# cryscan/bevy-hikari

Hardware: NVIDIA H100
Metric: Mrays/s (higher is better)
Workload: dtype f32

## Files before the change

bevy_hikari_b200/csrc/hk_device.cuh:

```cuda
#pragma once
#include <cuda_runtime.h>
#include <stdint.h>

#include "hikari_b200.h"
#include "hk_math.h"

#ifndef HK_INL_PACK
#define HK_INL_PACK __forceinline__
#endif
#ifndef HK_INL_TRAVERSE
#define HK_INL_TRAVERSE __forceinline__
#endif
#ifndef HK_INL_HITINFO
#define HK_INL_HITINFO __forceinline__
#endif
#ifndef HK_INL_TEXTURE
#define HK_INL_TEXTURE __forceinline__
#endif
#ifndef HK_SURFACE_LOOP
#define HK_SURFACE_LOOP 0
#endif
#ifndef HK_INL_SURFACE
#define HK_INL_SURFACE __forceinline__
#endif
// ... 516 lines not shown
        const uint32_t id0 = __float_as_uint(t0.x), id1 = __float_as_uint(t1.x), id2 = __float_as_uint(t1.w), id3 = __float_as_uint(t2.z);
#pragma unroll 1
        for (int k = 0; k < 4; ++k) {
            const uint32_t id = k == 0 ? id0 : (k == 1 ? id1 : (k == 2 ? id2 : id3));
            if (id == U32_MAX) continue;
            const vec4 t = sample_texture(sc, id, uv);
            if (k == 0) s.base_color = s.base_color * t;
            else if (k == 1) s.emissive = s.emissive * t;
            else if (k == 2) s.metallic *= t.x;
            else s.occlusion = t.x;
        }
#else
        uint32_t id = __float_as_uint(t0.x);
        if (id != U32_MAX) s.base_color = s.base_color * sample_texture(sc, id, uv);
        id = __float_as_uint(t1.x);
        if (id != U32_MAX) s.emissive = s.emissive * sample_texture(sc, id, uv);
        id = __float_as_uint(t1.w);
        if (id != U32_MAX) s.metallic *= sample_texture(sc, id, uv).x;
        id = __float_as_uint(t2.z);
        if (id != U32_MAX) s.occlusion = sample_texture(sc, id, uv).x;
#endif
    }
    s.roughness = perceptualRoughnessToRoughness(t1.y);
    s.reflectance = t2.x;
    return s;
}
static __device__ HK_INL_SURFACE vec4 retreive_emissive(const DeviceScene& sc, uint32_t material_index, vec2 uv) {
    const float4* m = reinterpret_cast<const float4*>(sc.materials + material_index);
    vec4 emissive = f4v(ldg4(m + 2));
    if (sc.texture_count != 0u) {
        uint32_t id = __float_as_uint(ldg4(m + 3).x);
        if (id != U32_MAX) emissive = emissive * sample_texture(sc, id, uv);
    }
    return emissive;
}

struct ShadeEnv {
    vec3 sun_dir; float cos_solar; vec3 sun_color; vec3 ambient; vec3 eye; bool ortho; vec3 ortho_dir;
};
__device__ __forceinline__ ShadeEnv make_env(const KParams& P) {
    ShadeEnv e;
    e.sun_dir = v3(P.in.lights.direction_to_light[0], P.in.lights.direction_to_light[1], P.in.lights.direction_to_light[2]);
    e.cos_solar = P.cos_solar_angle;
    e.sun_color = v3(P.in.lights.directional_color[0], P.in.lights.directional_color[1], P.in.lights.directional_color[2]);
    e.ambient = v3(P.in.lights.ambient_color[0], P.in.lights.ambient_color[1], P.in.lights.ambient_color[2]);
    e.eye = v3(P.in.view.world_position[0], P.in.view.world_position[1], P.in.view.world_position[2]);
    e.ortho = P.in.view.projection[15] == 1.0f;
    e.ortho_dir = v3(P.in.view.view_proj[2], P.in.view.view_proj[6], P.in.view.view_proj[10]);
    return e;
}
__device__ __forceinline__ vec3 calculate_view(const ShadeEnv& e, vec3 world_position) {
    return e.ortho ? normalize(e.ortho_dir) : normalize(e.eye - world_position);
}
__device__ __forceinline__ vec3 env_terms(vec3 diffuse_color, vec3 F0, float roughness, float NdotV) {
    return EnvBRDFApprox(diffuse_color, 1.0f, NdotV) + EnvBRDFApprox(F0, roughness, NdotV);
}
static __device__ HK_INL_SHADE vec3 env_brdf(vec3 V, vec3 N, const Surface& s) {
    vec3 base_color = xyz(s.base_color);
    float NdotV = fmax_(dot(N, V), 0.0001f);
    vec3 F0 = v3(0.16f * s.reflectance * s.reflectance * (1.0f - s.metallic)) + base_color * s.metallic;
    vec3 diffuse_color = base_color * (1.0f - s.metallic);
    return s.occlusion * env_terms(diffuse_color, F0, s.roughness, NdotV);
}
struct ShadeCtx {
    vec3 V, N, F0, diffuse_color, ambient_radiance;
    float roughness, NdotV, f90;
};
__device__ __forceinline__ ShadeCtx make_shade_ctx(const ShadeEnv& e, vec3 V, vec3 N, const Surface& s) {
    ShadeCtx c;
    vec3 base_color = xyz(s.base_color);
    c.V = V; c.N = N;
    c.F0 = v3(0.16f * s.reflectance * s.reflectance * (1.0f - s.metallic)) + base_color * s.metallic;
    c.diffuse_color = base_color * (1.0f - s.metallic);
    c.roughness = s.roughness;
    c.NdotV = fmax_(dot(N, V), 0.0001f);
    c.f90 = saturate(dot(c.F0, v3(50.0f * 0.33f)));
    c.ambient_radiance = s.occlusion * env_terms(c.diffuse_color, c.F0, s.roughness, c.NdotV) * e.ambient;
    return c;
}
__device__ __forceinline__ vec3 shade(const ShadeCtx& c, vec3 Lv, vec4 in_radiance) {
    vec3 Hv = normalize(Lv + c.V);
    float NoL = saturate(dot(c.N, Lv));
    float NoH = saturate(dot(c.N, Hv));
    float LoH = saturate(dot(Lv, Hv));
    vec3 diffuse = c.diffuse_color * Fd_Burley(c.roughness, c.NdotV, NoL, LoH);
    float D = D_GGX(c.roughness, NoH);
    float Vis = V_SmithGGXCorrelated(c.roughness, c.NdotV, NoL);
    vec3 F = F_Schlick_vec(c.F0, c.f90, LoH);
    vec3 specular_light = (1.0f * D * Vis) * F;
    vec3 lit_radiance = (specular_light + diffuse) * xyz(in_radiance) * NoL;
    return mix(lit_radiance, c.ambient_radiance, 1.0f - in_radiance.w);
}
static __device__ HK_INL_SHADE vec3 shading(const ShadeEnv& e, vec3 V, vec3 N, vec3 Lv, const Surface& s, vec4 in_radiance) {
    return shade(make_shade_ctx(e, V, N, s), Lv, in_radiance);
}
static __device__ HK_INL_RADIANCE vec4 input_radiance(const DeviceScene& sc, const ShadeEnv& e, vec3 ray_direction, const HitInfo& info,
                                               bool sample_directional, uint32_t sample_emissive, bool sample_ambient) {
    vec3 radiance = v3(0.0f);
    float amb = 0.0f;
    if (info.instance_index == U32_MAX) {
        bool hit_directional = dot(ray_direction, e.sun_dir) >= e.cos_solar;
        if (sample_directional && hit_directional) {
            radiance = e.sun_color;
        } else {
            radiance = sample_ambient ? e.ambient : v3(0.0f);
            amb = 1.0f;
        }
    } else if (sample_emissive == info.instance_index) {
        radiance = compute_emissive_radiance(retreive_emissive(sc, info.material_index, info.uv));
    }
    return v4(radiance, 1.0f - amb);
}

#ifndef HK_INL_WIDE
#define HK_INL_WIDE __forceinline__
#endif
template <bool BOTTOM>
static __device__ HK_INL_WIDE Hit wide_walk(const DeviceScene& sc, const Ray& ray, float max_distance, float early_distance,
                                            uint32_t exclude_instance, uint32_t instance);

template <bool COUNT_RAYS, bool WIDE = false>
static __device__ HK_INL_SELECT LightCandidate select_light_candidate(const DeviceScene& sc, const ShadeEnv& e, vec4 rnd, vec3 position,
                                                                 vec3 normal, uint32_t instance, HitInfo& info, uint32_t& blas_rays) {
    LightCandidate cand;
    cand.max_distance = F32_MAX;
    cand.min_distance = DISTANCE_MAX;
    cand.emissive_instance = DONT_SAMPLE_EMISSIVE;
    vec3 rand_direction = mul(normal_basis(e.sun_dir), sample_uniform_cone_dir(rnd.z, rnd.w, e.cos_solar));
    cand.direction = rand_direction;
    cand.p = 1.0f;
    info = empty_hit_info(position, rand_direction);
    if (instance == DONT_SAMPLE_EMISSIVE) return cand;

    uint32_t picked = U32_MAX;
    float count = 0.0f;
    float rand_1d = rnd.x;
    uint32_t index = 0;
    while (index < sc.emissive_node_count) {
        float4 n0 = ldg4(&sc.emissive_nodes[index]);
        uint32_t entry = __float_as_uint(n0.w);
        if (entry >= BVH_LEAF_FLAG) {
            uint32_t emissive_index = entry - BVH_LEAF_FLAG;
            float4 pr = ldg4(sc.emissives[emissive_index].position);
            uint32_t em_instance = __ldg(&sc.emissives[emissive_index].instance);
            vec3 c = f4xyz(pr);
            vec3 bmin = c - pr.w, bmax = c + pr.w;
            bool inside = position.x > bmin.x && position.y > bmin.y && position.z > bmin.z &&
                          position.x < bmax.x && position.y < bmax.y && position.z < bmax.z;
            if (instance != em_instance && inside) {
                rand_1d = fract(rand_1d + GOLDEN_RATIO);
                count += 1.0f;
                if (rand_1d < 1.0f / count) { cand.emissive_instance = em_instance; picked = emissive_index; }
            }
            index = __ldg(&sc.emissive_nodes[index].exit_index);
        } else {
            float4 n1 = ldg4(reinterpret_cast<const float4*>(&sc.emissive_nodes[index]) + 1);
            bool inside = position.x > n0.x && position.y > n0.y && position.z > n0.z &&
                          position.x < n1.x && position.y < n1.y && position.z < n1.z;
            index = inside ? entry : __float_as_uint(n1.w);
        }
    }

    if (cand.emissive_instance != DONT_SAMPLE_EMISSIVE) {
        const hk_emissive* em = sc.emissives + picked;
        uint4 e2 = ldg4u(&em->instance);
        float surface_area = __ldg(&em->surface_area);
        uint32_t alias_index = min(f32_to_u32(rnd.x * (float)e2.w), e2.w - 1u);
        uint2 ae = __ldg(reinterpret_cast<const uint2*>(sc.alias_table + e2.z + alias_index));
        uint32_t primitive_index = (rnd.y < __uint_as_float(ae.x)) ? ae.y : alias_index;

        const hk_instance* einst = sc.instances + cand.emissive_instance;
        uint4 mesh = ldg4u(&einst->mesh);
        const hk_primitive* prim = sc.primitives + mesh.y + primitive_index;
        vec3 p0 = f4xyz(ldg4(&prim->vertices[0])), p1 = f4xyz(ldg4(&prim->vertices[1])), p2 = f4xyz(ldg4(&prim->vertices[2]));
        float srx = sqrtf(rnd.z);
        float bx = 1.0f - srx, by = rnd.w * srx;
        vec3 lp = bx * p0 + by * p1 + (1.0f - bx - by) * p2;
        const float4* mm = reinterpret_cast<const float4*>(einst->model);
        mat4 model;
        model.c[0] = f4v(ldg4(mm)); model.c[1] = f4v(ldg4(mm + 1)); model.c[2] = f4v(ldg4(mm + 2)); model.c[3] = f4v(ldg4(mm + 3));
        vec4 wp = mul(model, v4(lp, 1.0f));
        vec3 p = xyz(wp) / wp.w;

        Hit hit;
        hit.u = 0.0f; hit.v = 0.0f; hit.distance = F32_MAX; hit.instance_index = U32_MAX; hit.primitive_index = U32_MAX;
        Ray ray;
        ray.origin = position + normal * RAY_BIAS;
        ray.direction = normalize(p - position);
        ray.inv_direction = v3(0.0f);
        cand.direction = ray.direction;
        bool found = false;
        if (dot(cand.direction, normal) > 0.0f) {
            if (COUNT_RAYS) blas_rays += 1u;
            Ray r;
            instance_ray(einst, ray, r);
            if constexpr (WIDE) {
                hit = wide_walk<true>(sc, r, F32_MAX, 0.0f, DONT_EXCLUDE, cand.emissive_instance);
                found = hit.primitive_index != U32_MAX;
            } else {
                found = traverse_bottom(sc, hit, r, mesh.y, mesh.z, mesh.w, 0.0f);
            }
        }
        if (found) {
            hit.instance_index = e2.x;
            info = hit_info(sc, ray, hit);
            cand.max_distance = hit.distance;
            cand.min_distance = hit.distance - 0.1f;
            vec3 delta = xyz(info.position) - position;
            cand.p = dot(delta, delta) / fabsf(dot(ray.direction, info.normal) * surface_area);
            cand.p = cand.p / count;
        } else {
            info = empty_hit_info(ray.origin, ray.direction);
            cand.emissive_instance = DONT_SAMPLE_EMISSIVE;
            cand.direction = rand_direction;
            cand.p = 1.0f;
        }
    }
    return cand;
}

__device__ __forceinline__ size_t band_index(const Band& b, int x, int y) { return (size_t)(y - b.a0) * (size_t)b.AW + (size_t)(x - b.ax0); }
__device__ __forceinline__ bool band_allocated(const Band& b, int x, int y) { return x >= b.ax0 && x < b.ax1 && y >= b.a0 && y < b.a1; }
__device__ __forceinline__ bool band_owned(const Band& b, int x, int y) { return x >= b.cx0 && x < b.cx1 && y >= b.r0 && y < b.r1; }
__device__ __forceinline__ size_t render_index(const Band& b, int x, int y) { return (size_t)(y - b.a0) * (size_t)b.RS + (size_t)(x - b.ax0); }
__device__ __forceinline__ size_t owned_index(const Band& b, int x, int y) { return (size_t)(y - b.r0) * (size_t)(b.cx1 - b.cx0) + (size_t)(x - b.cx0); }

__device__ __forceinline__ vec4 noise_random(const KParams& P, int x, int y) {
    uint32_t number = P.in.frame.number;
    uint32_t noise_id = number % NOISE_TEXTURE_COUNT;
    uint32_t tx = ((uint32_t)x + number) & 63u, ty = ((uint32_t)y + number) & 63u;
    uchar4 t = __ldg(reinterpret_cast<const uchar4*>(P.noise) + ((noise_id * 64u + ty) * 64u + tx));
    vec4 rnd = v4(unorm8(t.x), unorm8(t.y), unorm8(t.z), unorm8(t.w));
    return fract(rnd + (float)number * GOLDEN_RATIO);
}

__device__ __forceinline__ vec2 render_uv(const KParams& P, int x, int y) {
    return (v2((float)x, (float)y) + 0.5f) / v2((float)P.band.RW, (float)P.band.RH);
}
__device__ __forceinline__ vec2 jittered_deferred_uv(const KParams& P, vec2 uv, float amount) {
    if (P.ratio1) return uv;
    vec2 texel_size = v2(1.0f, 1.0f) / v2((float)P.band.W, (float)P.band.H);
    return uv + (P.jitter_sign * amount) * texel_size * P.ratio_m1;
}
__device__ __forceinline__ void light_deferred_coords(const KParams& P, vec2 uv, int x, int y, int& dx, int& dy) {
    if (P.ratio1) { dx = x; dy = y; return; }
    vec2 d = jittered_deferred_uv(P, uv, 0.25f);
    dx = f32_to_i32(d.x * (float)P.band.W); dy = f32_to_i32(d.y * (float)P.band.H);
}
__device__ __forceinline__ void denoise_deferred_coords(const KParams& P, vec2 uv, int x, int y, int& dx, int& dy) {
    if (P.ratio1) { dx = x; dy = y; return; }
    vec2 d = jittered_deferred_uv(P, uv, 0.5f);
    dx = min(max((int)floorf(d.x * (float)P.band.W), 0), P.band.W - 1);
    dy = min(max((int)floorf(d.y * (float)P.band.H), 0), P.band.H - 1);
}
__device__ __forceinline__ bool render_allocated(const KParams& P, int x, int y) {
    return P.ratio1 ? band_allocated(P.band, x, y) : (x >= 0 && x < P.band.RW && y >= 0 && y < P.band.RH);
}

struct PassBuffers {
    ReservoirPlanes previous_reservoir, reservoir, previous_spatial_reservoir, spatial_reservoir;
};
__device__ __forceinline__ PassBuffers bind(const KParams& P, int signal) {
    const int temporal = (signal == 0) ? 0 : (signal == 1 ? 2 : 6);
    const int spatial = (signal == 2) ? 8 : 4;
    const int current = (int)(P.in.frame.number & 1u), previous = 1 - current;
    PassBuffers b;
    b.previous_reservoir = P.planes.reservoir[current + temporal];
    b.reservoir = P.planes.reservoir[previous + temporal];
    b.previous_spatial_reservoir = P.planes.reservoir[current + spatial];
    b.spatial_reservoir = P.planes.reservoir[previous + spatial];
    return b;
}
__device__ __forceinline__ bool previous_pixel(const KParams& P, vec2 previous_uv, bool inclusive, size_t& pidx) {
    float ax = fabsf(previous_uv.x - 0.5f), ay = fabsf(previous_uv.y - 0.5f);
    bool inside = inclusive ? (ax <= 0.5f && ay <= 0.5f) : (ax < 0.5f && ay < 0.5f);
    if (!inside) return false;
    int px = f32_to_i32(previous_uv.x * (float)P.band.RW), py = f32_to_i32(previous_uv.y * (float)P.band.RH);
    if (!render_allocated(P, px, py)) return false;
    pidx = render_index(P.band, px, py);
    return true;
}
__device__ __forceinline__ vec2 pixel_uv(const KParams& P, int x, int y) { return render_uv(P, x, y); }
__device__ __forceinline__ size_t light_gbuffer_index(const KParams& P, int x, int y, size_t render_idx) {
    if (P.ratio1) return render_idx;
    int dx, dy;
    light_deferred_coords(P, render_uv(P, x, y), x, y, dx, dy);
    return band_index(P.band, dx, dy);
}

constexpr uint32_t SCATTER_BACKGROUND = 0u, SCATTER_MISS = 1u, SCATTER_VALIDATION = 2u;
__device__ __forceinline__ void scatter_claim(const KParams& P, size_t target, int x, int y, uint32_t kind) {
    uint32_t writer = (uint32_t)y * (uint32_t)P.band.RW + (uint32_t)x;
    atomicMax(&P.planes.scatter_key[target], ((writer + 1u) << 2) | kind);
}

#ifndef HK_CTA_WARPS
#define HK_CTA_WARPS 4
#endif
static_assert(HK_CTA_WARPS == 2 || HK_CTA_WARPS == 4 || HK_CTA_WARPS == 8, "tile_pixel places warps in pairs");
constexpr int TILE_W = 16, TILE_H = 2 * HK_CTA_WARPS, CTA_THREADS = 32 * HK_CTA_WARPS;
#ifndef HK_MINB_INDIRECT
#define HK_MINB_INDIRECT 8
#endif
#ifndef HK_MINB_DIRECT
#define HK_MINB_DIRECT 8
#endif
#ifndef HK_MINB_GBUFFER
#define HK_MINB_GBUFFER 8
#endif
#ifndef HK_MINB_INDIRECT_WIDE
#define HK_MINB_INDIRECT_WIDE 6
#endif
#ifndef HK_MINB_DIRECT_WIDE
#define HK_MINB_DIRECT_WIDE 6
#endif
#ifndef HK_MINB_DENOISE
#define HK_MINB_DENOISE 8
#endif
#ifndef HK_MINB_SPATIAL
#define HK_MINB_SPATIAL 8
#endif
__device__ __forceinline__ void tile_pixel(int& x, int& y, const KParams& P) {
    int lane = threadIdx.x & 31, warp = threadIdx.x >> 5;
    x = P.col_lo + blockIdx.x * TILE_W + (warp & 1) * 8 + (lane & 7);
    y = P.row_lo + blockIdx.y * TILE_H + (warp >> 1) * 4 + (lane >> 3);
}
__device__ __forceinline__ bool tile_active(const KParams& P, int x, int y) { return x < P.col_hi && y < P.row_hi; }

}
```

bevy_hikari_b200/csrc/kernels_light.cu:

```cuda
#include "hk_device.cuh"
#include "hk_wide.cuh"
#include "hk_kernels.h"

#ifndef HK_NO_TEXTURE_VARIANT
#define HK_NO_TEXTURE_VARIANT 1
#endif
#ifndef HK_NOVAL_VARIANT
#define HK_NOVAL_VARIANT 1
#endif

namespace hkd {

template <bool COUNT>
__device__ __forceinline__ void flush_counters(const KParams& P, uint32_t primary, uint32_t tlas, uint32_t blas) {
    if (!COUNT || P.counters == nullptr) return;
    for (int o = 16; o > 0; o >>= 1) {
        primary += __shfl_xor_sync(0xffffffffu, primary, o);
        tlas += __shfl_xor_sync(0xffffffffu, tlas, o);
        blas += __shfl_xor_sync(0xffffffffu, blas, o);
    }
    if ((threadIdx.x & 31) == 0) {
        if (primary) atomicAdd(&P.counters->primary, (unsigned long long)primary);
        if (tlas) atomicAdd(&P.counters->tlas, (unsigned long long)tlas);
        if (blas) atomicAdd(&P.counters->blas, (unsigned long long)blas);
    }
}

template <bool WIDE>
__device__ __forceinline__ Hit trace_top(const DeviceScene& sc, const Ray& ray, float max_distance, float early_distance, uint32_t exclude_instance) {
    if constexpr (WIDE) return wide_walk<false>(sc, ray, max_distance, early_distance, exclude_instance, 0u);
    else return traverse_top(sc, ray, max_distance, early_distance, exclude_instance);
}

__device__ __forceinline__ mat4 load_mat4(const float* m) {
    mat4 r;
    for (int c = 0; c < 4; ++c) r.c[c] = v4(m[4 * c], m[4 * c + 1], m[4 * c + 2], m[4 * c + 3]);
    return r;
}

__device__ __forceinline__ Ray primary_ray(const KParams& P, const mat4& inv_view_proj, float px, float py, vec2 jitter_ndc) {
    vec2 uv = v2(px + 0.5f, py + 0.5f) / v2((float)P.band.W, (float)P.band.H);
    vec2 ndc = v2(uv.x * 2.0f - 1.0f, (1.0f - uv.y) * 2.0f - 1.0f) - jitter_ndc;
    vec4 p = mul(inv_view_proj, v4(ndc.x, ndc.y, 1.0f, 1.0f));
    vec3 near_point = xyz(p) / p.w;
    Ray ray;
    if (P.in.view.projection[15] == 1.0f) {
        vec4 q = mul(inv_view_proj, v4(ndc.x, ndc.y, 0.0f, 1.0f));
        ray.origin = near_point;
        ray.direction = normalize(xyz(q) / q.w - near_point);
    } else {
        ray.origin = v3(P.in.view.world_position[0], P.in.view.world_position[1], P.in.view.world_position[2]);
        ray.direction = normalize(near_point - ray.origin);
    }
    ray.inv_direction = 1.0f / ray.direction;
    return ray;
}

template <bool TEX>
__device__ __forceinline__ DeviceScene scene_variant(const DeviceScene& scene) {
    DeviceScene sc = scene;
    if (!TEX) sc.texture_count = 0u;
    return sc;
}

template <bool COUNT, bool TEX = true, bool WIDE = false>
__global__ void __launch_bounds__(CTA_THREADS, HK_MINB_GBUFFER) k_gbuffer(const __grid_constant__ KParams P) {
    int x, y;
    tile_pixel(x, y, P);
    const bool active = tile_active(P, x, y);
    uint32_t n_primary = 0;
    if (active) {
        const size_t idx = band_index(P.band, x, y);
        const mat4 view_proj = load_mat4(P.in.view.view_proj);
        const mat4 inv_view_proj = load_mat4(P.in.view.inverse_view_proj);
        vec2 jitter_ndc = v2(0.0f, 0.0f);
        if (P.in.taa_jitter) {
            uint32_t index = P.in.smaa_tu4x ? ((P.in.frame.number >> 1u) & 15u) : (P.in.frame.number & 15u);
            const float* h = P.in.frame.halton[index >> 1u];
            vec2 hj = ((index & 1u) == 0u) ? v2(h[0], h[1]) : v2(h[2], h[3]);
            vec2 j = 2.0f * hj * (v2(1.0f, 1.0f) / v2(P.in.view.viewport[2], P.in.view.viewport[3]));
            jitter_ndc = v2(j.x, -j.y);
        }
        Ray ray = primary_ray(P, inv_view_proj, (float)x, (float)y, jitter_ndc);
        n_primary = 1;
        Hit hit = trace_top<WIDE>(P.scene, ray, F32_MAX, 0.0f, DONT_EXCLUDE);
        if (hit.instance_index == U32_MAX) {
            P.planes.pos_depth[idx] = make_float4(0.0f, 0.0f, 0.0f, 0.0f);
            P.planes.depth[idx] = 0.0f;
            P.planes.normal[idx] = 0u;
            P.planes.depth_gradient[idx] = make_float2(0.0f, 0.0f);
            P.planes.instance_material[idx] = make_float2(0.0f, 0.0f);
            P.planes.velocity_uv[idx] = make_float4(0.0f, 0.0f, 0.0f, 0.0f);
            P.planes.albedo[idx] = make_uint2(0u, 0u);
        } else {
            const DeviceScene sc = scene_variant<TEX>(P.scene);
            const hk_instance* inst = sc.instances + hit.instance_index;
            const hk_primitive* prim = sc.primitives + hit.primitive_index;
            uint32_t vbase = __ldg(&inst->mesh.vertex);
            uint32_t material = __ldg(&inst->material);
            float4 pa = ldg4(&prim->vertices[0]), pb = ldg4(&prim->vertices[1]), pc = ldg4(&prim->vertices[2]);
            const hk_vertex* va = sc.vertices + vbase + __float_as_uint(pa.w);
            const hk_vertex* vb = sc.vertices + vbase + __float_as_uint(pb.w);
            const hk_vertex* vc = sc.vertices + vbase + __float_as_uint(pc.w);
            float4 a0 = ldg4(va), a1 = ldg4(reinterpret_cast<const float4*>(va) + 1);
            float4 b0 = ldg4(vb), b1 = ldg4(reinterpret_cast<const float4*>(vb) + 1);
            float4 c0 = ldg4(vc), c1 = ldg4(reinterpret_cast<const float4*>(vc) + 1);
            vec3 world_position = ray.origin + ray.direction * hit.distance;
            vec4 clip = mul(view_proj, v4(world_position, 1.0f));
            float depth = clip.z / clip.w;
            vec3 n0 = instance_normal_local_to_world(inst, f4xyz(a1));
            vec3 n1 = instance_normal_local_to_world(inst, f4xyz(b1));
            vec3 n2 = instance_normal_local_to_world(inst, f4xyz(c1));
            vec3 world_normal = n0 + hit.u * (n1 - n0) + hit.v * (n2 - n0);
            vec2 uv0 = v2(a0.w, a1.w), uv1 = v2(b0.w, b1.w), uv2 = v2(c0.w, c1.w);
            vec2 tex_uv = uv0 + hit.u * (uv1 - uv0) + hit.v * (uv2 - uv0);
            const mat4 model = load_mat4(inst->model);
            vec3 P0 = xyz(mul(model, v4(f4xyz(pa), 1.0f)));
            vec3 P1 = xyz(mul(model, v4(f4xyz(pb), 1.0f)));
            vec3 P2 = xyz(mul(model, v4(f4xyz(pc), 1.0f)));
            vec3 Ng = cross(P1 - P0, P2 - P0);
            Ray rx = primary_ray(P, inv_view_proj, (float)x + 1.0f, (float)y, jitter_ndc);
            float tx = dot(P0 - rx.origin, Ng) / dot(rx.direction, Ng);
            vec4 cx = mul(view_proj, v4(rx.origin + rx.direction * tx, 1.0f));
            Ray ry = primary_ray(P, inv_view_proj, (float)x, (float)y + 1.0f, jitter_ndc);
            float ty = dot(P0 - ry.origin, Ng) / dot(ry.direction, Ng);
            vec4 cy = mul(view_proj, v4(ry.origin + ry.direction * ty, 1.0f));
            vec2 grad = v2(cx.z / cx.w - depth, cy.z / cy.w - depth);
            vec3 previous_world_position = world_position;
            if (sc.instance_moved != nullptr && __ldg(&sc.instance_moved[hit.instance_index]) != 0u) {
                const float4* pm = sc.previous_models + 4u * (size_t)hit.instance_index;
                mat4 previous_model;
                for (int c = 0; c < 4; ++c) previous_model.c[c] = f4v(ldg4(pm + c));
                vec3 local_position = f4xyz(pa) + hit.u * (f4xyz(pb) - f4xyz(pa)) + hit.v * (f4xyz(pc) - f4xyz(pa));
                previous_world_position = xyz(mul(previous_model, v4(local_position, 1.0f)));
            }
            vec4 pclip = mul(load_mat4(P.in.previous_view.view_proj), v4(previous_world_position, 1.0f));
            vec2 uva = v2(clip.x, clip.y) / clip.w; uva = (uva + 1.0f) * 0.5f; uva.y = 1.0f - uva.y;
            vec2 uvb = v2(pclip.x, pclip.y) / pclip.w; uvb = (uvb + 1.0f) * 0.5f; uvb.y = 1.0f - uvb.y;
            vec2 velocity = uva - uvb;
            uint32_t packed_normal = pack4x8snorm(v4(world_normal, 1.0f));
            P.planes.pos_depth[idx] = make_float4(world_position.x, world_position.y, world_position.z, depth);
            P.planes.depth[idx] = depth;
            P.planes.normal[idx] = packed_normal;
            P.planes.depth_gradient[idx] = make_float2(grad.x, grad.y);
            P.planes.instance_material[idx] = make_float2((float)hit.instance_index + 0.5f, (float)material + 0.5f);
            P.planes.velocity_uv[idx] = make_float4(velocity.x, velocity.y, tex_uv.x, tex_uv.y);
            uvec2 alb; alb.x = 0u; alb.y = 0u;
            if (!(depth < F32_EPSILON)) {
                ShadeEnv env = make_env(P);
                vec3 normal = xyz(unpack4x8snorm(packed_normal));
                Surface surface = retreive_surface(sc, f32_to_u32((float)material + 0.5f), tex_uv);
                vec3 view_direction = calculate_view(env, world_position);
                alb = pack_rgba16f(v4(env_brdf(view_direction, normal, surface), 1.0f));
            }
            P.planes.albedo[idx] = make_uint2(alb.x, alb.y);
        }
    }
    if (!band_owned(P.band, x, y)) n_primary = 0;
    flush_counters<COUNT>(P, n_primary, 0u, 0u);
}

__global__ void __launch_bounds__(CTA_THREADS) k_albedo(const __grid_constant__ KParams P) {
    int x, y;
    tile_pixel(x, y, P);
    if (!tile_active(P, x, y)) return;
    const size_t idx = band_index(P.band, x, y);
    float4 pd = P.planes.pos_depth[idx];
    P.planes.depth[idx] = pd.w;
    if (pd.w < F32_EPSILON) { P.planes.albedo[idx] = make_uint2(0u, 0u); return; }
    ShadeEnv env = make_env(P);
    vec3 normal = xyz(unpack4x8snorm(P.planes.normal[idx]));
    float2 im = P.planes.instance_material[idx];
    float4 vu = P.planes.velocity_uv[idx];
    Surface surface = retreive_surface(P.scene, f32_to_u32(im.y), v2(vu.z, vu.w));
    uvec2 alb = pack_rgba16f(v4(env_brdf(calculate_view(env, f4xyz(pd)), normal, surface), 1.0f));
    P.planes.albedo[idx] = make_uint2(alb.x, alb.y);
}

template <bool EMISSIVE_LIT, bool COUNT, bool TEX = true, bool NOVAL = false, bool WIDE = false>
__global__ void __launch_bounds__(CTA_THREADS, WIDE ? HK_MINB_DIRECT_WIDE : HK_MINB_DIRECT) k_direct(const __grid_constant__ KParams P) {
    constexpr int SIGNAL = EMISSIVE_LIT ? 1 : 0;
    constexpr bool RENDER_EMISSIVE = !EMISSIVE_LIT;
    int x, y;
    tile_pixel(x, y, P);
    const bool active = tile_active(P, x, y);
    uint32_t n_tlas = 0, n_blas = 0;
    if (active) {
        const DeviceScene sc = scene_variant<TEX>(P.scene);
        const hk_frame_uniform& frame = P.in.frame;
        const size_t idx = render_index(P.band, x, y);
        const size_t gidx = light_gbuffer_index(P, x, y, idx);
        const PassBuffers B = bind(P, SIGNAL);
        const float4 pd = P.planes.pos_depth[gidx];
        const float depth = pd.w;
        if (depth < F32_EPSILON) {
            Reservoir r = zero_reservoir();
            set_reservoir(r, zero_sample(), 0.0f);
            PackedQuarters q = pack_reservoir(r);
            store_quarters(B.reservoir, idx, q);
            store_quarters(B.spatial_reservoir, idx, q);
            scatter_claim(P, idx, x, y, SCATTER_BACKGROUND);
            P.planes.variance[SIGNAL][idx] = 0.0f;
            P.planes.render[SIGNAL][idx] = make_uint2(0u, 0u);
        } else {
            const ShadeEnv env = make_env(P);
            const vec3 position = f4xyz(pd);
            const vec3 normal = xyz(unpack4x8snorm(P.planes.normal[gidx]));
            const float2 imf = P.planes.instance_material[gidx];
            const uint32_t instance_id = f32_to_u32(imf.x), material_id = f32_to_u32(imf.y);
            const float4 vu = P.planes.velocity_uv[gidx];

            Sample s = zero_sample();
            s.random = noise_random(P, x, y);
            s.visible_position = v4(position, depth);
            s.visible_normal = normal;
            s.visible_instance = instance_id;

            HitInfo info = empty_hit_info(v3(0.0f), v3(0.0f));
            info.instance_index = 0u; info.material_index = 0u; info.position = v4(0.0f);

            const vec2 previous_uv = jittered_deferred_uv(P, pixel_uv(P, x, y), 0.25f) - v2(vu.x, vu.y);
            size_t pidx = 0;
            Reservoir r = zero_reservoir();
            if (previous_pixel(P, previous_uv, false, pidx)) r = unpack_reservoir(load_quarters(B.previous_reservoir, pidx));
            if (!check_previous_reservoir(r, s)) {
                size_t sidx;
                if (previous_pixel(P, previous_uv, true, sidx)) scatter_claim(P, sidx, x, y, SCATTER_MISS);
            }

            const uint32_t validate_interval = EMISSIVE_LIT ? frame.emissive_validate_interval : frame.direct_validate_interval;
            const uint32_t select_light_instance = EMISSIVE_LIT ? instance_id : DONT_SAMPLE_EMISSIVE;
            const bool validation_frame = NOVAL ? false : (frame.number % validate_interval) == 0u;

            if (!validation_frame || r.count < 4.0f) {
                LightCandidate cand = select_light_candidate<COUNT, WIDE>(sc, env, s.random, position, normal, select_light_instance, info, n_blas);
                Ray ray;
                ray.origin = position + normal * RAY_BIAS;
                ray.direction = cand.direction;
                ray.inv_direction = 1.0f / ray.direction;
                bool trace_condition = dot(cand.direction, normal) > 0.0f && cand.p > 0.0f;
                if (EMISSIVE_LIT) trace_condition = trace_condition && cand.emissive_instance != DONT_SAMPLE_EMISSIVE;
                if (trace_condition) {
                    if (COUNT) n_tlas += 1u;
                    Hit hit = trace_top<WIDE>(sc, ray, cand.max_distance, cand.min_distance, cand.emissive_instance);
                    occlude_hit_info(ray, hit, info);
                    s.radiance = EMISSIVE_LIT ? input_radiance(sc, env, ray.direction, info, false, cand.emissive_instance, false)
                                              : input_radiance(sc, env, ray.direction, info, true, DONT_SAMPLE_EMISSIVE, false);
                }
                s.sample_position = info.position;
                s.sample_normal = info.normal;
                float w_new = (cand.p > 0.0f) ? luminance(xyz(s.radiance)) / cand.p : 0.0f;
                temporal_restir(r, s, w_new, frame.max_temporal_reuse_count);
            }

            if (validation_frame) {
                LightCandidate cand = select_light_candidate<COUNT, WIDE>(sc, env, r.s.random, xyz(r.s.visible_position), r.s.visible_normal,
                                                                    select_light_instance, info, n_blas);
                Ray ray;
                ray.origin = position + normal * RAY_BIAS;
                ray.direction = normalize(xyz(r.s.sample_position) - position);
                ray.inv_direction = 1.0f / ray.direction;
                vec4 validate_radiance = v4(0.0f);
                bool trace_condition = dot(cand.direction, r.s.visible_normal) > 0.0f && cand.p > 0.0f;
                if (EMISSIVE_LIT) trace_condition = trace_condition && cand.emissive_instance != DONT_SAMPLE_EMISSIVE;
                if (trace_condition) {
                    if (COUNT) n_tlas += 1u;
                    Hit hit = trace_top<WIDE>(sc, ray, cand.max_distance, cand.min_distance, cand.emissive_instance);
                    occlude_hit_info(ray, hit, info);
                    validate_radiance = EMISSIVE_LIT ? input_radiance(sc, env, ray.direction, info, false, cand.emissive_instance, false)
                                                     : input_radiance(sc, env, ray.direction, info, true, DONT_SAMPLE_EMISSIVE, false);
                }
                if (r.count >= 4.0f) {
                    s.random = r.s.random;
                    s.sample_position = info.position;
                    s.sample_normal = info.normal;
                    s.radiance = validate_radiance;
                }
                float luminance_ratio = luminance(xyz(validate_radiance)) / fmax_(luminance(xyz(r.s.radiance)), 0.0001f);
                if (luminance_ratio > 1.25f || luminance_ratio < 0.8f) {
                    size_t sidx;
                    if (previous_pixel(P, previous_uv, true, sidx)) {
                        store_quarters(P.planes.scatter_value, idx, pack_reservoir(r));
                        scatter_claim(P, sidx, x, y, SCATTER_VALIDATION);
                    }
                    float w_new = (cand.p > 0.0f) ? luminance(xyz(s.radiance)) / cand.p : 0.0f;
                    set_reservoir(r, s, w_new);
                }
            }

            float total_lum = r.count * luminance(xyz(r.s.radiance));
            r.w = (total_lum > 0.0f) ? r.w_sum / total_lum : 0.0f;
            r.s.visible_position = s.visible_position;
            r.s.visible_normal = s.visible_normal;
            r.lifetime += 1.0f;
            P.planes.variance[SIGNAL][idx] = variance_of(r);
            if (frame.temporal_reuse > 0u) store_quarters(B.reservoir, idx, pack_reservoir(r));

            Surface surface = retreive_surface(sc, material_id, v2(vu.z, vu.w));
            vec3 view_direction = calculate_view(env, position);
            vec3 out_radiance = shading(env, view_direction, r.s.visible_normal,
                                        normalize(xyz(r.s.sample_position) - xyz(r.s.visible_position)), surface, r.s.radiance);
            out_radiance = out_radiance * r.w;
            vec3 out_color = RENDER_EMISSIVE ? out_radiance + compute_emissive_radiance(surface.emissive) : out_radiance;
            uvec2 o = pack_rgba16f(v4(out_color, 1.0f));
            P.planes.render[SIGNAL][idx] = make_uint2(o.x, o.y);
        }
    }
    if (!band_owned(P.band, x, y)) { n_tlas = 0; n_blas = 0; }
    flush_counters<COUNT>(P, 0u, n_tlas, n_blas);
}

template <bool MULTI, bool COUNT, bool TEX = true, bool WIDE = false>
__global__ void __launch_bounds__(CTA_THREADS, WIDE ? HK_MINB_INDIRECT_WIDE : HK_MINB_INDIRECT) k_indirect(const __grid_constant__ KParams P) {
    int x, y;
    tile_pixel(x, y, P);
    const bool active = tile_active(P, x, y);
    uint32_t n_tlas = 0, n_blas = 0;
    if (active) {
        const DeviceScene sc = scene_variant<TEX>(P.scene);
        const hk_frame_uniform& frame = P.in.frame;
        const size_t idx = render_index(P.band, x, y);
        const size_t gidx = light_gbuffer_index(P, x, y, idx);
        const PassBuffers B = bind(P, 2);
        const float4 pd = P.planes.pos_depth[gidx];
        const float depth = pd.w;
        if (frame.indirect_bounces == 0u || depth < F32_EPSILON) {
            PackedQuarters q = pack_reservoir(zero_reservoir());
            store_quarters(B.reservoir, idx, q);
            store_quarters(B.spatial_reservoir, idx, q);
            scatter_claim(P, idx, x, y, SCATTER_BACKGROUND);
            P.planes.variance[2][idx] = 0.0f;
            P.planes.render[2][idx] = make_uint2(0u, 0u);
        } else {
            const ShadeEnv env = make_env(P);
            const vec3 position = f4xyz(pd);
            const vec3 normal = normalize(xyz(unpack4x8snorm(P.planes.normal[gidx])));
            const float2 imf = P.planes.instance_material[gidx];
            const uint32_t instance_id = f32_to_u32(imf.x), material_id = f32_to_u32(imf.y);
            const float4 vu = P.planes.velocity_uv[gidx];

            Sample s = zero_sample();
            s.random = noise_random(P, x, y);
            s.visible_position = v4(position, depth);
            s.visible_normal = normal;
            s.visible_instance = instance_id;

            float pdf = 0.0f;
            vec3 b_position = position, b_normal = normal;
            vec4 b_random = s.random;
            vec3 color_transport = v3(1.0f);
            const uint32_t bounces = MULTI ? frame.indirect_bounces : 1u;
            for (uint32_t n = 0u; n < bounces && (color_transport.x > 0.01f || color_transport.y > 0.01f || color_transport.z > 0.01f); n += 1u) {
                vec4 rand_sample = sample_cosine_hemisphere(b_random.x, b_random.y);
                Ray ray;
                ray.origin = b_position + b_normal * RAY_BIAS;
                ray.direction = mul(normal_basis(b_normal), xyz(rand_sample));
                ray.inv_direction = 1.0f / ray.direction;
                if (COUNT) n_tlas += 1u;
                Hit hit = trace_top<WIDE>(sc, ray, F32_MAX, 0.0f, DONT_EXCLUDE);
                HitInfo info = hit_info(sc, ray, hit);
                if (n == 0u) {
                    s.sample_position = info.position;
                    s.sample_normal = info.normal;
                    pdf = rand_sample.w;
                }
                const vec3 h_position = xyz(info.position), h_normal = info.normal;
                if (hit.instance_index != U32_MAX) {
                    vec3 out_radiance = v3(0.0f);
                    Surface surface = retreive_surface(sc, info.material_index, info.uv);
                    surface.roughness = 1.0f;
                    LightCandidate cand = select_light_candidate<COUNT, WIDE>(sc, env, b_random, h_position, h_normal, info.instance_index, info, n_blas);
                    const bool sample_directional = (cand.emissive_instance == DONT_SAMPLE_EMISSIVE);
                    const vec3 bounce_view_direction = normalize(b_position - h_position);
                    if (dot(cand.direction, h_normal) > 0.0f && cand.p > 0.0f) {
                        ray.origin = h_position + h_normal * RAY_BIAS;
                        ray.direction = cand.direction;
                        ray.inv_direction = 1.0f / ray.direction;
                        if (COUNT) n_tlas += 1u;
                        hit = trace_top<WIDE>(sc, ray, cand.max_distance, cand.min_distance, cand.emissive_instance);
                        occlude_hit_info(ray, hit, info);
                        vec4 in_radiance = input_radiance(sc, env, ray.direction, info, sample_directional, cand.emissive_instance, false);
                        out_radiance = shading(env, bounce_view_direction, h_normal, ray.direction, surface, in_radiance);
                        out_radiance = out_radiance / cand.p;
                        if (MULTI) {
                            if (n > 0u) out_radiance = (rand_sample.w < 0.01f) ? v3(0.0f) : out_radiance / rand_sample.w;
                            float out_luminance = luminance(out_radiance);
                            if (out_luminance > frame.max_indirect_luminance)
                                out_radiance = out_radiance * frame.max_indirect_luminance / out_luminance;
                            s.radiance = s.radiance + v4(color_transport * out_radiance, 1.0f);
                        } else {
                            s.radiance = s.radiance + v4(out_radiance, 1.0f);
                        }
                    }
                    if (MULTI) {
                        color_transport = color_transport * env_brdf(bounce_view_direction, h_normal, surface);
                        b_random = fract(b_random + (float)frame.number * GOLDEN_RATIO);
                        b_position = h_position;
                        b_normal = h_normal;
                    }
                } else {
                    vec3 out_radiance = xyz(input_radiance(sc, env, ray.direction, info, false, DONT_SAMPLE_EMISSIVE, true));
                    s.radiance = MULTI ? s.radiance + v4(color_transport * out_radiance, 0.0f) : s.radiance + v4(out_radiance, 0.0f);
                    break;
                }
            }

            const vec2 previous_uv = jittered_deferred_uv(P, pixel_uv(P, x, y), 0.25f) - v2(vu.x, vu.y);
            size_t pidx = 0;
            Reservoir r = zero_reservoir();
            if (previous_pixel(P, previous_uv, false, pidx)) r = unpack_reservoir(load_quarters(B.previous_reservoir, pidx));
            if (!check_previous_reservoir(r, s)) {
                size_t sidx;
                if (previous_pixel(P, previous_uv, true, sidx)) scatter_claim(P, sidx, x, y, SCATTER_MISS);
            }
            Surface surface = retreive_surface(sc, material_id, v2(vu.z, vu.w));
            vec3 view_direction = calculate_view(env, position);
            vec3 sample_radiance = shading(env, view_direction, s.visible_normal,
                                           normalize(xyz(s.sample_position) - xyz(s.visible_position)), surface, s.radiance);
            float w_new = (pdf > 0.0f) ? luminance(sample_radiance) / pdf : 0.0f;
            temporal_restir(r, s, w_new, frame.max_temporal_reuse_count);

            vec3 out_radiance = shading(env, view_direction, r.s.visible_normal,
                                        normalize(xyz(r.s.sample_position) - xyz(r.s.visible_position)), surface, r.s.radiance);
            float total_lum = r.count * luminance(out_radiance);
            r.w = (total_lum > 0.0f) ? r.w_sum / total_lum : 0.0f;
            r.s.visible_position = s.visible_position;
            r.s.visible_normal = s.visible_normal;
            r.lifetime += 1.0f;
            P.planes.variance[2][idx] = variance_of(r);
            if (frame.temporal_reuse > 0u) store_quarters(B.reservoir, idx, pack_reservoir(r));
            uvec2 o = pack_rgba16f(v4(out_radiance * r.w, 1.0f));
            P.planes.render[2][idx] = make_uint2(o.x, o.y);
        }
    }
    if (!band_owned(P.band, x, y)) { n_tlas = 0; n_blas = 0; }
    flush_counters<COUNT>(P, 0u, n_tlas, n_blas);
}

__global__ void __launch_bounds__(CTA_THREADS) k_extract_depth(const __grid_constant__ KParams P) {
    int x, y;
    tile_pixel(x, y, P);
    if (!tile_active(P, x, y)) return;
    const size_t idx = band_index(P.band, x, y);
    P.planes.depth[idx] = P.planes.pos_depth[idx].w;
}

__global__ void __launch_bounds__(CTA_THREADS) k_scatter_resolve(const __grid_constant__ KParams P, int signal) {
    int x, y;
    tile_pixel(x, y, P);
    if (!tile_active(P, x, y)) return;
    const size_t idx = render_index(P.band, x, y);
    const uint32_t key = P.planes.scatter_key[idx];
    if (key == 0u) return;
    P.planes.scatter_key[idx] = 0u;
    const uint32_t kind = key & 3u, writer = (key >> 2) - 1u;
    const PassBuffers B = bind(P, signal);
    PackedQuarters q;
    if (kind == SCATTER_VALIDATION) {
        const int wy = (int)(writer / (uint32_t)P.band.RW), wx = (int)(writer % (uint32_t)P.band.RW);
        q = load_quarters(P.planes.scatter_value, render_index(P.band, wx, wy));
    } else {
        Reservoir r = zero_reservoir();
        if (kind == SCATTER_BACKGROUND && signal != 2) set_reservoir(r, zero_sample(), 0.0f);
        q = pack_reservoir(r);
    }
    store_quarters(B.previous_spatial_reservoir, idx, q);
}

template <bool WIDE>
__global__ void k_trace_rays(DeviceScene sc, const hk_ray* rays, size_t n, hk_hit* hits) {
    size_t i = (size_t)blockIdx.x * blockDim.x + threadIdx.x;
    if (i >= n) return;
    Ray r;
    r.origin = v3(rays[i].origin[0], rays[i].origin[1], rays[i].origin[2]);
    r.direction = v3(rays[i].direction[0], rays[i].direction[1], rays[i].direction[2]);
    r.inv_direction = 1.0f / r.direction;
    Hit h = trace_top<WIDE>(sc, r, rays[i].max_distance, rays[i].early_distance, rays[i].exclude_instance);
    hits[i].u = h.u; hits[i].v = h.v; hits[i].distance = h.distance;
    hits[i].instance_index = h.instance_index; hits[i].primitive_index = h.primitive_index;
}

static dim3 grid_for(const KParams& P) {
    int rows = P.row_hi - P.row_lo, cols = P.col_hi - P.col_lo;
    return dim3((unsigned)((cols + TILE_W - 1) / TILE_W), (unsigned)((rows + TILE_H - 1) / TILE_H), 1u);
}

}

using namespace hkd;

static inline bool no_texture(const KParams& P) { return HK_NO_TEXTURE_VARIANT && P.scene.texture_count == 0u; }
static inline bool wide_mode(const KParams& P, bool wide) { return wide && P.scene.wide_ready != 0u; }

void hk_launch_gbuffer(const KParams& P, bool count, bool wide, cudaStream_t st) {
    if (P.row_hi <= P.row_lo || P.col_hi <= P.col_lo) return;
    const dim3 g = grid_for(P);
    if (wide_mode(P, wide)) {
        if (count) k_gbuffer<true, true, true><<<g, CTA_THREADS, 0, st>>>(P);
        else if (no_texture(P)) k_gbuffer<false, false, true><<<g, CTA_THREADS, 0, st>>>(P);
        else k_gbuffer<false, true, true><<<g, CTA_THREADS, 0, st>>>(P);
        return;
    }
    if (count) k_gbuffer<true><<<g, CTA_THREADS, 0, st>>>(P);
    else if (no_texture(P)) k_gbuffer<false, false><<<g, CTA_THREADS, 0, st>>>(P);
    else k_gbuffer<false><<<g, CTA_THREADS, 0, st>>>(P);
}
void hk_launch_extract_depth(const KParams& P, cudaStream_t st) {
    if (P.row_hi <= P.row_lo || P.col_hi <= P.col_lo) return;
    k_extract_depth<<<grid_for(P), CTA_THREADS, 0, st>>>(P);
}
void hk_launch_albedo(const KParams& P, cudaStream_t st) {
    if (P.row_hi <= P.row_lo || P.col_hi <= P.col_lo) return;
    k_albedo<<<grid_for(P), CTA_THREADS, 0, st>>>(P);
}
template <bool WIDE>
static void launch_direct(const KParams& P, bool emissive, bool count, cudaStream_t st) {
    dim3 g = grid_for(P);
    const uint32_t interval = emissive ? P.in.frame.emissive_validate_interval : P.in.frame.direct_validate_interval;
    const bool noval = HK_NOVAL_VARIANT && !count && (P.in.frame.number % interval) != 0u;
    if (noval) {
        if (no_texture(P)) {
            if (emissive) k_direct<true, false, false, true, WIDE><<<g, CTA_THREADS, 0, st>>>(P);
            else k_direct<false, false, false, true, WIDE><<<g, CTA_THREADS, 0, st>>>(P);
        } else {
            if (emissive) k_direct<true, false, true, true, WIDE><<<g, CTA_THREADS, 0, st>>>(P);
            else k_direct<false, false, true, true, WIDE><<<g, CTA_THREADS, 0, st>>>(P);
        }
        return;
    }
    if (!count && no_texture(P)) {
        if (emissive) k_direct<true, false, false, false, WIDE><<<g, CTA_THREADS, 0, st>>>(P);
        else k_direct<false, false, false, false, WIDE><<<g, CTA_THREADS, 0, st>>>(P);
        return;
    }
    if (emissive) { if (count) k_direct<true, true, true, false, WIDE><<<g, CTA_THREADS, 0, st>>>(P); else k_direct<true, false, true, false, WIDE><<<g, CTA_THREADS, 0, st>>>(P); }
    else { if (count) k_direct<false, true, true, false, WIDE><<<g, CTA_THREADS, 0, st>>>(P); else k_direct<false, false, true, false, WIDE><<<g, CTA_THREADS, 0, st>>>(P); }
}
void hk_launch_direct(const KParams& P, bool emissive, bool count, bool wide, cudaStream_t st) {
    if (P.row_hi <= P.row_lo || P.col_hi <= P.col_lo) return;
    if (wide_mode(P, wide)) launch_direct<true>(P, emissive, count, st);
    else launch_direct<false>(P, emissive, count, st);
}
template <bool WIDE>
static void launch_indirect(const KParams& P, bool multi, bool count, cudaStream_t st) {
    dim3 g = grid_for(P);
    if (!count && no_texture(P)) {
        if (multi) k_indirect<true, false, false, WIDE><<<g, CTA_THREADS, 0, st>>>(P);
        else k_indirect<false, false, false, WIDE><<<g, CTA_THREADS, 0, st>>>(P);
        return;
    }
    if (multi) { if (count) k_indirect<true, true, true, WIDE><<<g, CTA_THREADS, 0, st>>>(P); else k_indirect<true, false, true, WIDE><<<g, CTA_THREADS, 0, st>>>(P); }
    else { if (count) k_indirect<false, true, true, WIDE><<<g, CTA_THREADS, 0, st>>>(P); else k_indirect<false, false, true, WIDE><<<g, CTA_THREADS, 0, st>>>(P); }
}
void hk_launch_indirect(const KParams& P, bool multi, bool count, bool wide, cudaStream_t st) {
    if (P.row_hi <= P.row_lo || P.col_hi <= P.col_lo) return;
    if (wide_mode(P, wide)) launch_indirect<true>(P, multi, count, st);
    else launch_indirect<false>(P, multi, count, st);
}
void hk_launch_scatter_resolve(const KParams& P, int signal, cudaStream_t st) {
    if (P.row_hi <= P.row_lo || P.col_hi <= P.col_lo) return;
    k_scatter_resolve<<<grid_for(P), CTA_THREADS, 0, st>>>(P, signal);
}
void hk_launch_trace_rays(const DeviceScene& sc, const hk_ray* rays, size_t n, hk_hit* hits, bool wide, cudaStream_t st) {
    if (n == 0) return;
    if (wide && sc.wide_ready != 0u) k_trace_rays<true><<<(unsigned)((n + 127) / 128), 128, 0, st>>>(sc, rays, n, hits);
    else k_trace_rays<false><<<(unsigned)((n + 127) / 128), 128, 0, st>>>(sc, rays, n, hits);
}
```

Baseline: 1715.

## Split indirect kernel into path-tracing and ReSTIR resolve kernels

Splits the monolithic indirect lighting kernel in two. The first traces the path and writes radiance and the first-hit sample to the scatter_value scratch planes. The second runs the temporal ReSTIR reuse and shading with its own launch bound. The aim is to lower register pressure in the traversal kernel so more warps fit on each SM. The cost is an extra launch plus a write and re-read of three 16-byte values per pixel, and it reuses scatter_value planes that other passes may also depend on.

```diff
diff --git a/bevy_hikari_b200/csrc/hk_device.cuh b/bevy_hikari_b200/csrc/hk_device.cuh
--- a/bevy_hikari_b200/csrc/hk_device.cuh
+++ b/bevy_hikari_b200/csrc/hk_device.cuh
@@ -842,6 +842,9 @@
 #ifndef HK_MINB_INDIRECT
 #define HK_MINB_INDIRECT 8
 #endif
+#ifndef HK_MINB_INDIRECT_RESTIR
+#define HK_MINB_INDIRECT_RESTIR 5
+#endif
 #ifndef HK_MINB_DIRECT
 #define HK_MINB_DIRECT 8
 #endif
diff --git a/bevy_hikari_b200/csrc/kernels_light.cu b/bevy_hikari_b200/csrc/kernels_light.cu
--- a/bevy_hikari_b200/csrc/kernels_light.cu
+++ b/bevy_hikari_b200/csrc/kernels_light.cu
@@ -310,44 +310,47 @@
     flush_counters<COUNT>(P, 0u, n_tlas, n_blas);
 }
 
+struct PathResult { vec4 radiance, sample_position; vec3 sample_normal; float pdf; };
+__device__ __forceinline__ void store_path_sample(const KParams& P, size_t idx, vec4 sample_position, vec3 sample_normal, float pdf) {
+    P.planes.scatter_value.q[1][idx] = make_uint4(__float_as_uint(sample_position.x), __float_as_uint(sample_position.y),
+                                                  __float_as_uint(sample_position.z), __float_as_uint(sample_position.w));
+    P.planes.scatter_value.q[2][idx] = make_uint4(__float_as_uint(sample_normal.x), __float_as_uint(sample_normal.y),
+                                                  __float_as_uint(sample_normal.z), __float_as_uint(pdf));
+}
+__device__ __forceinline__ void store_path_radiance(const KParams& P, size_t idx, vec4 radiance) {
+    P.planes.scatter_value.q[0][idx] = make_uint4(__float_as_uint(radiance.x), __float_as_uint(radiance.y),
+                                                  __float_as_uint(radiance.z), __float_as_uint(radiance.w));
+}
+__device__ __forceinline__ PathResult load_path(const KParams& P, size_t idx) {
+    const uint4 a = P.planes.scatter_value.q[0][idx], b = P.planes.scatter_value.q[1][idx], c = P.planes.scatter_value.q[2][idx];
+    PathResult r;
+    r.radiance = v4(__uint_as_float(a.x), __uint_as_float(a.y), __uint_as_float(a.z), __uint_as_float(a.w));
+    r.sample_position = v4(__uint_as_float(b.x), __uint_as_float(b.y), __uint_as_float(b.z), __uint_as_float(b.w));
+    r.sample_normal = v3(__uint_as_float(c.x), __uint_as_float(c.y), __uint_as_float(c.z));
+    r.pdf = __uint_as_float(c.w);
+    return r;
+}
+__device__ __forceinline__ bool indirect_background(const KParams& P, float depth) {
+    return P.in.frame.indirect_bounces == 0u || depth < F32_EPSILON;
+}
+
 template <bool MULTI, bool COUNT, bool TEX = true, bool WIDE = false>
-__global__ void __launch_bounds__(CTA_THREADS, WIDE ? HK_MINB_INDIRECT_WIDE : HK_MINB_INDIRECT) k_indirect(const __grid_constant__ KParams P) {
+__global__ void __launch_bounds__(CTA_THREADS, WIDE ? HK_MINB_INDIRECT_WIDE : HK_MINB_INDIRECT) k_indirect_path(const __grid_constant__ KParams P) {
     int x, y;
     tile_pixel(x, y, P);
     const bool active = tile_active(P, x, y);
     uint32_t n_tlas = 0, n_blas = 0;
     if (active) {
-        const DeviceScene sc = scene_variant<TEX>(P.scene);
-        const hk_frame_uniform& frame = P.in.frame;
         const size_t idx = render_index(P.band, x, y);
         const size_t gidx = light_gbuffer_index(P, x, y, idx);
-        const PassBuffers B = bind(P, 2);
         const float4 pd = P.planes.pos_depth[gidx];
-        const float depth = pd.w;
-        if (frame.indirect_bounces == 0u || depth < F32_EPSILON) {
-            PackedQuarters q = pack_reservoir(zero_reservoir());
-            store_quarters(B.reservoir, idx, q);
-            store_quarters(B.spatial_reservoir, idx, q);
-            scatter_claim(P, idx, x, y, SCATTER_BACKGROUND);
-            P.planes.variance[2][idx] = 0.0f;
-            P.planes.render[2][idx] = make_uint2(0u, 0u);
-        } else {
+        if (!indirect_background(P, pd.w)) {
+            const DeviceScene sc = scene_variant<TEX>(P.scene);
+            const hk_frame_uniform& frame = P.in.frame;
             const ShadeEnv env = make_env(P);
-            const vec3 position = f4xyz(pd);
-            const vec3 normal = normalize(xyz(unpack4x8snorm(P.planes.normal[gidx])));
-            const float2 imf = P.planes.instance_material[gidx];
-            const uint32_t instance_id = f32_to_u32(imf.x), material_id = f32_to_u32(imf.y);
-            const float4 vu = P.planes.velocity_uv[gidx];
-
-            Sample s = zero_sample();
-            s.random = noise_random(P, x, y);
-            s.visible_position = v4(position, depth);
-            s.visible_normal = normal;
-            s.visible_instance = instance_id;
-
-            float pdf = 0.0f;
-            vec3 b_position = position, b_normal = normal;
-            vec4 b_random = s.random;
+            vec4 radiance = v4(0.0f);
+            vec3 b_position = f4xyz(pd), b_normal = normalize(xyz(unpack4x8snorm(P.planes.normal[gidx])));
+            vec4 b_random = noise_random(P, x, y);
             vec3 color_transport = v3(1.0f);
             const uint32_t bounces = MULTI ? frame.indirect_bounces : 1u;
             for (uint32_t n = 0u; n < bounces && (color_transport.x > 0.01f || color_transport.y > 0.01f || color_transport.z > 0.01f); n += 1u) {
@@ -359,11 +362,7 @@
                 if (COUNT) n_tlas += 1u;
                 Hit hit = trace_top<WIDE>(sc, ray, F32_MAX, 0.0f, DONT_EXCLUDE);
                 HitInfo info = hit_info(sc, ray, hit);
-                if (n == 0u) {
-                    s.sample_position = info.position;
-                    s.sample_normal = info.normal;
-                    pdf = rand_sample.w;
-                }
+                if (n == 0u) store_path_sample(P, idx, info.position, info.normal, rand_sample.w);
                 const vec3 h_position = xyz(info.position), h_normal = info.normal;
                 if (hit.instance_index != U32_MAX) {
                     vec3 out_radiance = v3(0.0f);
@@ -387,9 +386,9 @@
                             float out_luminance = luminance(out_radiance);
                             if (out_luminance > frame.max_indirect_luminance)
                                 out_radiance = out_radiance * frame.max_indirect_luminance / out_luminance;
-                            s.radiance = s.radiance + v4(color_transport * out_radiance, 1.0f);
+                            radiance = radiance + v4(color_transport * out_radiance, 1.0f);
                         } else {
-                            s.radiance = s.radiance + v4(out_radiance, 1.0f);
+                            radiance = radiance + v4(out_radiance, 1.0f);
                         }
                     }
                     if (MULTI) {
@@ -400,41 +399,82 @@
                     }
                 } else {
                     vec3 out_radiance = xyz(input_radiance(sc, env, ray.direction, info, false, DONT_SAMPLE_EMISSIVE, true));
-                    s.radiance = MULTI ? s.radiance + v4(color_transport * out_radiance, 0.0f) : s.radiance + v4(out_radiance, 0.0f);
+                    radiance = MULTI ? radiance + v4(color_transport * out_radiance, 0.0f) : radiance + v4(out_radiance, 0.0f);
                     break;
                 }
             }
-
-            const vec2 previous_uv = jittered_deferred_uv(P, pixel_uv(P, x, y), 0.25f) - v2(vu.x, vu.y);
-            size_t pidx = 0;
-            Reservoir r = zero_reservoir();
-            if (previous_pixel(P, previous_uv, false, pidx)) r = unpack_reservoir(load_quarters(B.previous_reservoir, pidx));
-            if (!check_previous_reservoir(r, s)) {
-                size_t sidx;
-                if (previous_pixel(P, previous_uv, true, sidx)) scatter_claim(P, sidx, x, y, SCATTER_MISS);
-            }
-            Surface surface = retreive_surface(sc, material_id, v2(vu.z, vu.w));
-            vec3 view_direction = calculate_view(env, position);
-            vec3 sample_radiance = shading(env, view_direction, s.visible_normal,
-                                           normalize(xyz(s.sample_position) - xyz(s.visible_position)), surface, s.radiance);
-            float w_new = (pdf > 0.0f) ? luminance(sample_radiance) / pdf : 0.0f;
-            temporal_restir(r, s, w_new, frame.max_temporal_reuse_count);
-
-            vec3 out_radiance = shading(env, view_direction, r.s.visible_normal,
-                                        normalize(xyz(r.s.sample_position) - xyz(r.s.visible_position)), surface, r.s.radiance);
-            float total_lum = r.count * luminance(out_radiance);
-            r.w = (total_lum > 0.0f) ? r.w_sum / total_lum : 0.0f;
-            r.s.visible_position = s.visible_position;
-            r.s.visible_normal = s.visible_normal;
-            r.lifetime += 1.0f;
-            P.planes.variance[2][idx] = variance_of(r);
-            if (frame.temporal_reuse > 0u) store_quarters(B.reservoir, idx, pack_reservoir(r));
-            uvec2 o = pack_rgba16f(v4(out_radiance * r.w, 1.0f));
-            P.planes.render[2][idx] = make_uint2(o.x, o.y);
+            store_path_radiance(P, idx, radiance);
         }
     }
     if (!band_owned(P.band, x, y)) { n_tlas = 0; n_blas = 0; }
     flush_counters<COUNT>(P, 0u, n_tlas, n_blas);
+}
+
+template <bool TEX = true>
+__global__ void __launch_bounds__(CTA_THREADS, HK_MINB_INDIRECT_RESTIR) k_indirect_restir(const __grid_constant__ KParams P) {
+    int x, y;
+    tile_pixel(x, y, P);
+    if (!tile_active(P, x, y)) return;
+    const DeviceScene sc = scene_variant<TEX>(P.scene);
+    const hk_frame_uniform& frame = P.in.frame;
+    const size_t idx = render_index(P.band, x, y);
+    const size_t gidx = light_gbuffer_index(P, x, y, idx);
+    const PassBuffers B = bind(P, 2);
+    const float4 pd = P.planes.pos_depth[gidx];
+    const float depth = pd.w;
+    if (indirect_background(P, depth)) {
+        PackedQuarters q = pack_reservoir(zero_reservoir());
+        store_quarters(B.reservoir, idx, q);
+        store_quarters(B.spatial_reservoir, idx, q);
+        scatter_claim(P, idx, x, y, SCATTER_BACKGROUND);
+        P.planes.variance[2][idx] = 0.0f;
+        P.planes.render[2][idx] = make_uint2(0u, 0u);
+    } else {
+        const ShadeEnv env = make_env(P);
+        const vec3 position = f4xyz(pd);
+        const vec3 normal = normalize(xyz(unpack4x8snorm(P.planes.normal[gidx])));
+        const float2 imf = P.planes.instance_material[gidx];
+        const uint32_t instance_id = f32_to_u32(imf.x), material_id = f32_to_u32(imf.y);
+        const float4 vu = P.planes.velocity_uv[gidx];
+
+        const PathResult path = load_path(P, idx);
+        Sample s = zero_sample();
+        s.random = noise_random(P, x, y);
+        s.visible_position = v4(position, depth);
+        s.visible_normal = normal;
+        s.visible_instance = instance_id;
+        s.radiance = path.radiance;
+        s.sample_position = path.sample_position;
+        s.sample_normal = path.sample_normal;
+        const float pdf = path.pdf;
+
+        const vec2 previous_uv = jittered_deferred_uv(P, pixel_uv(P, x, y), 0.25f) - v2(vu.x, vu.y);
+        size_t pidx = 0;
+        Reservoir r = zero_reservoir();
+        if (previous_pixel(P, previous_uv, false, pidx)) r = unpack_reservoir(load_quarters(B.previous_reservoir, pidx));
+        if (!check_previous_reservoir(r, s)) {
+            size_t sidx;
+            if (previous_pixel(P, previous_uv, true, sidx)) scatter_claim(P, sidx, x, y, SCATTER_MISS);
+        }
+        Surface surface = retreive_surface(sc, material_id, v2(vu.z, vu.w));
+        vec3 view_direction = calculate_view(env, position);
+        vec3 sample_radiance = shading(env, view_direction, s.visible_normal,
+                                       normalize(xyz(s.sample_position) - xyz(s.visible_position)), surface, s.radiance);
+        float w_new = (pdf > 0.0f) ? luminance(sample_radiance) / pdf : 0.0f;
+        temporal_restir(r, s, w_new, frame.max_temporal_reuse_count);
+
+        vec3 out_radiance = shading(env, view_direction, r.s.visible_normal,
+                                    normalize(xyz(r.s.sample_position) - xyz(r.s.visible_position)), surface, r.s.radiance);
+        float total_lum = r.count * luminance(out_radiance);
+        r.w = (total_lum > 0.0f) ? r.w_sum / total_lum : 0.0f;
+        r.s.visible_position = s.visible_position;
+        r.s.visible_normal = s.visible_normal;
+        r.lifetime += 1.0f;
+        P.planes.variance[2][idx] = variance_of(r);
+        if (frame.temporal_reuse > 0u) store_quarters(B.reservoir, idx, pack_reservoir(r));
+        uvec2 o = pack_rgba16f(v4(out_radiance * r.w, 1.0f));
+        P.planes.render[2][idx] = make_uint2(o.x, o.y);
+    }
 }
 
 __global__ void __launch_bounds__(CTA_THREADS) k_extract_depth(const __grid_constant__ KParams P) {
@@ -545,12 +585,14 @@
 static void launch_indirect(const KParams& P, bool multi, bool count, cudaStream_t st) {
     dim3 g = grid_for(P);
     if (!count && no_texture(P)) {
-        if (multi) k_indirect<true, false, false, WIDE><<<g, CTA_THREADS, 0, st>>>(P);
-        else k_indirect<false, false, false, WIDE><<<g, CTA_THREADS, 0, st>>>(P);
+        if (multi) k_indirect_path<true, false, false, WIDE><<<g, CTA_THREADS, 0, st>>>(P);
+        else k_indirect_path<false, false, false, WIDE><<<g, CTA_THREADS, 0, st>>>(P);
+        k_indirect_restir<false><<<g, CTA_THREADS, 0, st>>>(P);
         return;
     }
-    if (multi) { if (count) k_indirect<true, true, true, WIDE><<<g, CTA_THREADS, 0, st>>>(P); else k_indirect<true, false, true, WIDE><<<g, CTA_THREADS, 0, st>>>(P); }
-    else { if (count) k_indirect<false, true, true, WIDE><<<g, CTA_THREADS, 0, st>>>(P); else k_indirect<false, false, true, WIDE><<<g, CTA_THREADS, 0, st>>>(P); }
+    if (multi) { if (count) k_indirect_path<true, true, true, WIDE><<<g, CTA_THREADS, 0, st>>>(P); else k_indirect_path<true, false, true, WIDE><<<g, CTA_THREADS, 0, st>>>(P); }
+    else { if (count) k_indirect_path<false, true, true, WIDE><<<g, CTA_THREADS, 0, st>>>(P); else k_indirect_path<false, false, true, WIDE><<<g, CTA_THREADS, 0, st>>>(P); }
+    k_indirect_restir<true><<<g, CTA_THREADS, 0, st>>>(P);
 }
 void hk_launch_indirect(const KParams& P, bool multi, bool count, bool wide, cudaStream_t st) {
     if (P.row_hi <= P.row_lo || P.col_hi <= P.col_lo) return;
```

Result: faster. 1794, median of 6 (+4.6%).
